# junwenxiong/diff_sal

Hardware: AMD Instinct MI355X
Metric: denoise-steps/sec (batch x NFE / wall time), 16x224x384 clip, 50-step DPM-Solver (higher is better)
Workload: dtype f32; 1 GPU; BASELINE configs[1]: DHF1k visual-only, batch=4/GPU, 224x384, 50-NFE DPM-Solver (multistep-2, logSNR, denoise-to-zero), faithful full graph; batch_per_gpu=4, nfe_per_trajectory=50, step=one SalUNet evaluation + DPM-Solver update on one batch, sampler_mode=eager

## Files before the change

diff_sal_amd/csrc/common.h:

```cpp
#pragma once
#include <hip/hip_runtime.h>

#include <cstdarg>
#include <cstdint>
#include <cstdio>

#include "../../include/diffsal.h"

namespace diffsal {

void set_error(const char* fmt, ...);
void note_kernel(const char* fmt, ...);

inline bool aligned16(const void* p) { return (reinterpret_cast<uintptr_t>(p) & 15u) == 0; }

inline int check_launch(const char* what) {
  hipError_t e = hipGetLastError();
  if (e != hipSuccess) {
    set_error("%s: launch failed: %s", what, hipGetErrorString(e));
    return DIFFSAL_E_LAUNCH;
  }
  return DIFFSAL_OK;
}

#define DS_REQUIRE(cond, code, ...)  \
  do {                               \
    if (!(cond)) {                   \
      diffsal::set_error(__VA_ARGS__); \
      return (code);                 \
    }                                \
  } while (0)

constexpr int kWave = 64;

#define DIFFSAL_TUNE_KEYS(X) \
  X(NO_PERSIST) X(NO_XCD_ORDER) X(NO_HALO) X(FORCE_HALO) X(IGEMM_CFG) X(IGEMM16_CFG) X(PLAN_DEBUG) \
  X(WGRAD_CFG) X(WGRAD_SPLITS) X(WGRAD_VERBOSE) X(NO_FUSED_BLOCK) X(NO_WINOGRAD) X(FORCE_WINOGRAD) X(GN_CHUNKS) \
  X(GN_APPLY_WGS) X(GEMM_DMA) X(CONV_DMA) X(GROUP_GRID) X(GEMM_DMA16) X(WGRAD_DMA) X(NO_GN_SLAB) X(NO_WINOGRAD4) X(BATCH_TILE) \
  X(BATCH_XCD) X(NO_TAPSUM_ROWS) X(TAPSUM_ROWS_FORM) X(NO_ATTN_BWD_DS) X(NO_POOL_RUNS) X(NO_ATTN_SLOTS) X(NO_STREAM16) \
  X(CONV16_TILE) X(BLOCK16_WAVES) X(NO_ATTN16_MFMA) X(CONV16_HALF) X(FRONT_FOLD_WGS)
#define DIFFSAL_TUNE_ENUM(name) TUNE_##name,
enum TuneKey { DIFFSAL_TUNE_KEYS(DIFFSAL_TUNE_ENUM) TUNE_COUNT };
#undef DIFFSAL_TUNE_ENUM
int tune(int key);

template <int CTRL>
__device__ __forceinline__ float dpp_move(float v) {
  return __builtin_bit_cast(float, __builtin_amdgcn_update_dpp(0, __builtin_bit_cast(int, v), CTRL, 0xF, 0xF, false));
}
__device__ __forceinline__ float lane_xor16(float v) {
  const unsigned u = __builtin_bit_cast(unsigned, v);
  const auto r = __builtin_amdgcn_permlane16_swap(u, u, false, false);
  return __builtin_bit_cast(float, (__lane_id() & 16) ? r[0] : r[1]);
}
__device__ __forceinline__ float lane_xor32(float v) {
  const unsigned u = __builtin_bit_cast(unsigned, v);
  const auto r = __builtin_amdgcn_permlane32_swap(u, u, false, false);
  return __builtin_bit_cast(float, (__lane_id() & 32) ? r[0] : r[1]);
}
template <int WIDTH, typename OP>
__device__ __forceinline__ float group_reduce(float v, OP op) {
  static_assert(WIDTH >= 1 && WIDTH <= 64 && (WIDTH & (WIDTH - 1)) == 0, "power of two <= 64");
  if constexpr (WIDTH >= 2) v = op(v, dpp_move<0xB1>(v));
  if constexpr (WIDTH >= 4) v = op(v, dpp_move<0x4E>(v));
  if constexpr (WIDTH >= 8) v = op(v, dpp_move<0x141>(v));
  if constexpr (WIDTH >= 16) v = op(v, dpp_move<0x140>(v));
  if constexpr (WIDTH >= 32) v = op(v, lane_xor16(v));
  if constexpr (WIDTH >= 64) v = op(v, lane_xor32(v));
  return v;
}
template <int WIDTH>
__device__ __forceinline__ float group_sum(float v) {
  return group_reduce<WIDTH>(v, [](float a, float b) { return a + b; });
// ... 295 lines not shown
```

diff_sal_amd/csrc/gemm_dma.hip:

```cpp
#include <type_traits>

#include "common.h"

namespace diffsal {

struct DmaGemmArgs {
  const void* a;
  const void* w;
  const float* bias;
  const float* scale;
  const float* shift;
  const float* rowvec;
  const void* residual;
  void* out;
  int M, N, K;
  int act, rowvec_ld, rows_per_img;
  int n_tiles_m, n_tiles_n, n_tiles;
  int xcd_order;
  int H, W, Cin, Ho, Wo, KW, taps, stride_h, stride_w, pad_t, pad_l, dil_h, dil_w;
  unsigned in_bytes;
  int splits, kt_per_unit;
  float* partial;
  int batch;
  long a_bs, w_bs, o_bs;
// ... 502 lines not shown
    stamp(3 + 3 * t);
    cmp_v += gsz;
  }
}

template <typename T>
__global__ __launch_bounds__(256) void gemm_dma_reduce_kernel(DmaGemmArgs p) {
  const T* __restrict__ resid = static_cast<const T*>(p.residual);
  T* __restrict__ outp = static_cast<T*>(p.out);
  const int n4 = p.N >> 2;
  const long total = static_cast<long>(p.M) * n4, slab = static_cast<long>(p.M) * p.N;
  for (long i = static_cast<long>(blockIdx.x) * 256 + threadIdx.x; i < total; i += static_cast<long>(gridDim.x) * 256) {
    const int n = static_cast<int>(i % n4) * 4;
    const long m = i / n4, o = m * p.N + n;
    float4 a = ld4(p.partial + o);
    for (int s = 1; s < p.splits; ++s) {
      const float4 b = ld4(p.partial + s * slab + o);
      a.x += b.x; a.y += b.y; a.z += b.z; a.w += b.w;
    }
    float v[4] = {a.x, a.y, a.z, a.w};
#pragma unroll
    for (int e = 0; e < 4; ++e) {
      float x[1] = {v[e]};
      epi_channels(x, p.bias, p.scale, p.shift, p.rowvec, [&] { return (m / p.rows_per_img) * p.rowvec_ld; }, n + e);
      epi_act(x, p.act);
      v[e] = x[0];
    }
    if (p.act == DIFFSAL_ACT_GELU_GRAD) epi_gelu_grad(v, ld4(resid + o));
    else if (resid) epi_add(v, ld4(resid + o));
    st4(outp + o, make_float4(v[0], v[1], v[2], v[3]));
  }
}

namespace {

int choose_split(long tiles, int kt, int stages, long mn, double* t_out = nullptr) {
  int best = 1;
  double best_t = 1e30;
  for (int S = 1; S <= 32; ++S) {
    if (kt % (S * stages) != 0) continue;
    const int per = kt / S;
    if (S > 1 && per < 2 * stages) break;
    const long units = tiles * S;
    const double rounds = static_cast<double>((units + 255) / 256);
    double t = rounds * per * 1.13e-6;
    t += 3.0e-6 + 1.2e-6;
    if (S > 1) t += (S + 1.0) * mn * 4.0 / 3.0e12 + 4.0e-6;
    if (t < best_t) { best_t = t; best = S; }
  }
  if (t_out) *t_out = best_t;
  return best;
}

template <typename T, int TMB, int TNB, int STAGES, int OCC>
int launch_dma(DmaGemmArgs& a, bool conv, hipStream_t s) {
  constexpr int BM = 32 * TMB, BN = 32 * TNB;
  const int slots = 256 * OCC;
  const int units = a.n_tiles * a.splits * (a.batch + a.batch2);
  const int grid = units < slots ? units : slots;
#ifdef DIFFSAL_DEV_STAMPS
  a.stamps = (g_dma_stamps && static_cast<size_t>(grid) * 32 * 8 <= g_dma_stamp_bytes) ? g_dma_stamps : nullptr;
#endif
  const long rows_total = static_cast<long>(a.n_tiles_m) * (a.batch + a.batch2);
  const bool batched = a.batch + a.batch2 > 1;
  a.xcd_order = (a.splits == 1 && tune(TUNE_NO_XCD_ORDER) != 1 && grid % 8 == 0 && a.n_tiles_n > 1 &&
                 (batched ? (tune(TUNE_BATCH_XCD) == 1 && units >= 128 && rows_total >= 16) : (a.n_tiles >= slots && a.n_tiles_m >= 16))) ? 1 : 0;
// ... 93 lines not shown
  else rc = launch_dma<f16_t, 3, 3, 3, 2>(g, false, s);
  return rc == DIFFSAL_OK ? 1 : rc;
}

int gemm_dma_batched(const float* a, const float* w, float* out, long M, int K, int N, int batch, long a_bs, long w_bs, long o_bs,
                     hipStream_t s, const float* side_a, const float* side_w, float* side_out, long side_rows) {
  diffsal_conv_desc d{};
  d.N = 1; d.H = 1; d.W = static_cast<int>(M); d.Ho = 1; d.Wo = static_cast<int>(M); d.Cin = K; d.Cout = N; d.KH = 1; d.KW = 1;
  d.stride_h = d.stride_w = d.dil_h = d.dil_w = 1;
  d.dtype = DIFFSAL_F32;
  if (M <= 0 || M >= (1L << 31) || batch < 1 || a_bs % 4 != 0 || w_bs % 4 != 0 || o_bs % 4 != 0) return 0;
  const long nb2 = side_rows > 0 ? side_rows / M : 0;
  if (side_rows > 0 && (side_rows % M != 0 || !side_a || !side_w || !side_out || !aligned16(side_a) || !aligned16(side_w) ||
                        !aligned16(side_out) || nb2 > 4096))
    return 0;
  const long tm = (M + 95) / 96, nbt = batch + nb2;
  const long u96 = tm * ((N + 95) / 96) * nbt, u128 = tm * ((N + 127) / 128) * nbt;
  const double t96 = static_cast<double>((u96 + 255) / 256), t128 = static_cast<double>((u128 + 255) / 256) * (4.0 / 3.0);
  const int force = tune(TUNE_BATCH_TILE);
  const bool wide = N % 128 == 0 && (force == 1 || (force != 0 && t128 * 1.1 < t96));
  DmaGemmArgs g;
  if (!dma_fill(g, kDmaCfgs[wide ? 2 : 0], &d, false, 4, a, w, nullptr, nullptr, nullptr, nullptr, 0, nullptr, out)) return 0;
  g.batch = batch; g.a_bs = a_bs; g.w_bs = w_bs; g.o_bs = o_bs;
  if (side_rows > 0) {
    g.batch2 = static_cast<int>(nb2);
    g.a2 = side_a; g.w2 = side_w; g.out2 = side_out;
    g.a2_bs = M * K; g.o2_bs = M * N;
  }
  if (static_cast<long>(g.n_tiles) * (batch + g.batch2) >= (1L << 30)) return 0;
  const int rc = wide ? launch_dma<float, 3, 4, 3, 1>(g, false, s) : launch_dma<float, 3, 3, 3, 2>(g, false, s);
  return rc == DIFFSAL_OK ? 1 : rc;
}

int try_gemm_dma_group(int n, const diffsal_conv_desc* const* d, const float* const* a, const float* const* w, const float* const* bias,
                       float* const* out, hipStream_t s) {
  if (n < 1 || n > kMaxGroup) return 0;
  const DmaCfg& c = kDmaCfgs[0];
  DmaGemmArgs pr[kMaxGroup];
  for (int i = 0; i < n; ++i)
    if (!dma_fill(pr[i], c, d[i], true, 4, a[i], w[i], bias ? bias[i] : nullptr, nullptr, nullptr, nullptr, 0, nullptr, out[i])) return 0;
  int order[kMaxGroup];
  for (int i = 0; i < n; ++i) order[i] = i;
  for (int i = 0; i < n; ++i)
    for (int j = i + 1; j < n; ++j)
      if (pr[order[j]].kt_per_unit > pr[order[i]].kt_per_unit) { const int t = order[i]; order[i] = order[j]; order[j] = t; }
  DmaGroupArgs g{};
  g.n = n;
  int units = 0;
  for (int i = 0; i < kMaxGroup; ++i) {
    if (i < n) {
      g.prob[i] = pr[order[i]];
      units += g.prob[i].n_tiles;
    } else {
      g.prob[i] = g.prob[n - 1];
    }
    g.unit_end[i] = i < n ? units : 0x7FFFFFFF;
  }
  g.total = units;
  const int persist = tune(TUNE_GROUP_GRID);
  const int grid = persist > 0 && units > persist ? persist : units;
  hipLaunchKernelGGL((gemm_dma_kernel<float, 3, 3, 3, 2, true, true>), dim3(grid), dim3(256), 0, s, g);
  note_kernel("gemm_dma_kernel<float, 3, 3, 3, 2, true, true> [96x96 tile, 3 stages, %d problems, %d units]", n, units);
  const int rc = check_launch("diffsal_conv_igemm_group(dma)");
  return rc == DIFFSAL_OK ? 1 : rc;
}

}

#ifdef DIFFSAL_DEV_STAMPS
extern "C" int diffsal_set_dma_stamps(void* device_buffer, size_t bytes) {
  diffsal::g_dma_stamps = static_cast<unsigned long long*>(device_buffer);
  diffsal::g_dma_stamp_bytes = device_buffer ? bytes : 0;
  return DIFFSAL_OK;
}
#endif
```

diff_sal_amd/csrc/igemm.hip:

```cpp
#include <cstdlib>
#include <type_traits>

#include "common.h"

namespace diffsal {

size_t igemm16_ws_bytes(const diffsal_conv_desc* d);
int igemm16_launch(const diffsal_conv_desc* d, const void* in, const void* w, const float* bias, const float* scale,
                   const float* shift, const float* rowvec, const void* residual, void* out, void* ws, size_t ws_bytes,
                   hipStream_t s, const void* in2 = nullptr, const void* w2 = nullptr, const float* bias2 = nullptr,
                   void* out2 = nullptr);

int try_linear_stream(const float* x, const float* w, const float* bias, const float* residual, float* out, long M,
                      int K, int N, int act, hipStream_t s);

int try_gemm_dma(int cfg, const diffsal_conv_desc* d, bool as_conv, const void* a, const void* w, const float* bias, const float* scale,
                 const float* shift, const float* rowvec, int rowvec_ld, const void* residual, void* out, void* ws, size_t ws_bytes,
                 hipStream_t s, bool out_f32 = false);
int try_gemm_dma_group(int n, const diffsal_conv_desc* const* d, const float* const* a, const float* const* w, const float* const* bias,
                       float* const* out, hipStream_t s);
size_t gemm_dma_ws_bytes(int cfg, long M, int K, int N, int esz);
int try_gemm16_dma2(const diffsal_conv_desc* d, const void* a, const void* w, const float* bias, const float* scale, const float* shift,
                    const float* rowvec, int rowvec_ld, const void* residual, void* out, hipStream_t s, bool out_f32);
double gemm_dma_estimate(int cfg, long M, int K, int N);

struct IgemmArgs {
  const float* in;
  const float* w;
  const float* bias;
  const float* scale;
  const float* shift;
  const float* rowvec;
  const float* residual;
  float* out;
  int M, K;
  int H, W, Cin, Ho, Wo, Cout;
  int KW, taps, stride_h, stride_w, pad_t, pad_l, dil_h, dil_w;
  int act, rowvec_ld;
  int linear;
  int persist_wgs;
  int w_split;
  int n_tiles_n, n_tiles;
  unsigned in_bytes, w_bytes;
  int splits, kt_per_split;
  float* partial;
  int vec_epilogue;
  int xcd_order;
  int pair;
  const float* in2;
  const float* w2;
  const float* bias2;
  float* out2;
  float* partial2;
// ... 705 lines not shown
  g = g > 2048 ? 2048 : g;
  hipLaunchKernelGGL(splitk_reduce_kernel, dim3(static_cast<int>(g), nz), dim3(256), 0, s, a);
  return check_launch("diffsal_conv_igemm(split-K reduce)");
}

}

using namespace diffsal;

static int dma_route(const diffsal_conv_desc* d, bool linear, long M, int K, bool pair) {
  if (d->precision != DIFFSAL_PREC_FP32 || d->w_format != 0 || pair) return -1;
  if (d->dtype != DIFFSAL_F32) {
    if (!linear || tune(TUNE_IGEMM16_CFG) >= 0 || K % 192 != 0 || d->Cout % 4 != 0) return -1;
    const int forced = tune(TUNE_GEMM_DMA16);
    if (forced == 0) return -1;
    if (forced > 0) return forced == 2 ? 3 : 0;
    return ((M + 95) / 96) * ((d->Cout + 95) / 96) >= 192 ? 0 : -1;
  }
  if (tune(TUNE_IGEMM_CFG) >= 0) return -1;
  const long tiles96 = ((M + 95) / 96) * ((d->Cout + 95) / 96);
  if (linear) {
    const int forced = tune(TUNE_GEMM_DMA);
    if (forced == 0) return -1;
    if (forced > 0) return forced - 1;
    if (K % 96 != 0 || d->Cout % 4 != 0) return -1;
    const double t_dma = gemm_dma_estimate(0, M, K, d->Cout);
    const double t_tiled = choose_plan(M, d->Cout, K, d->precision, true).t;
    return t_dma <= 1.25 * t_tiled ? 0 : -1;
  }
  const int forced = tune(TUNE_CONV_DMA);
  if (forced == 0) return -1;
  if (forced > 0) return forced - 1;
  if (K % 96 != 0 || d->Cout % 4 != 0) return -1;
  return ((tiles96 >= 1024 && K <= 1024) || (M <= 400 && K >= 3072)) ? 0 : -1;
}

static int validate(const diffsal_conv_desc* d) {
  DS_REQUIRE(d, DIFFSAL_E_ARG, "conv_igemm: null descriptor");
  DS_REQUIRE(d->Cin > 0 && d->Cin % 32 == 0, DIFFSAL_E_SHAPE, "conv_igemm: Cin=%d must be a multiple of 32", d->Cin);
  DS_REQUIRE(d->N > 0 && d->H > 0 && d->W > 0 && d->Cout > 0 && d->KH > 0 && d->KW > 0 && d->stride_h > 0 &&
                 d->stride_w > 0 && d->dil_h > 0 && d->dil_w > 0,
             DIFFSAL_E_SHAPE, "conv_igemm: non-positive dimension");
  DS_REQUIRE(d->Ho > 0 && d->Wo > 0, DIFFSAL_E_SHAPE, "conv_igemm: empty output %dx%d", d->Ho, d->Wo);
  const long M = static_cast<long>(d->N) * d->Ho * d->Wo;
  DS_REQUIRE(M < (1L << 31) && M * d->Cout < (1L << 40), DIFFSAL_E_SHAPE, "conv_igemm: problem too large");
  DS_REQUIRE(d->KH * d->KW <= 32, DIFFSAL_E_SHAPE, "conv_igemm: at most 32 taps (KH*KW=%d)", d->KH * d->KW);
  DS_REQUIRE(d->precision == DIFFSAL_PREC_FP32 || d->precision == DIFFSAL_PREC_BF16X3, DIFFSAL_E_ARG,
             "conv_igemm: precision %d (DIFFSAL_PREC_FP32 or DIFFSAL_PREC_BF16X3)", d->precision);
  DS_REQUIRE(d->dtype == DIFFSAL_F32 || d->dtype == DIFFSAL_BF16 || d->dtype == DIFFSAL_F16, DIFFSAL_E_ARG,
             "conv_igemm: dtype %d (DIFFSAL_F32, DIFFSAL_BF16 or DIFFSAL_F16)", d->dtype);
  DS_REQUIRE(d->dtype == DIFFSAL_F32 || (d->precision == DIFFSAL_PREC_FP32 && d->w_format == 0), DIFFSAL_E_ARG,
             "conv_igemm: 16-bit storage uses the native MFMA (precision and w_format must be 0)");
  const long esz = d->dtype == DIFFSAL_F32 ? 4 : 2;
  const long in_bytes = static_cast<long>(d->N) * d->H * d->W * d->Cin * esz;
  const long w_bytes = static_cast<long>(d->Cout) * d->KH * d->KW * d->Cin * esz;
  DS_REQUIRE(in_bytes < (1L << 32) - 16 && w_bytes < (1L << 32) - 16, DIFFSAL_E_SHAPE,
             "conv_igemm: input (%ld B) and weight (%ld B) must each stay below 4 GiB (32-bit buffer offsets); "
             "split the batch", in_bytes, w_bytes);
  return DIFFSAL_OK;
}

static Plan plan_or_forced(long M, int Cout, int K, int precision, bool linear) {
  Plan pl = choose_plan(M, Cout, K, precision, linear);
  const int v = tune(TUNE_IGEMM_CFG);
  if (v >= 0) {
    pl.cfg = (v % 8) % kNumCfgs;
    pl.splits = 1;
// ... 111 lines not shown
  a.kt_per_split = (a.K / BK + pl.splits - 1) / pl.splits;
  a.partial = nullptr;
  if (pl.splits > 1) {
    const size_t one = static_cast<size_t>(pl.splits) * M * d->Cout * sizeof(float);
    const size_t need = px ? 2 * one : one;
    DS_REQUIRE(ws && ws_bytes >= need && aligned16(ws) && aligned16(out), DIFFSAL_E_ARG,
               "conv_igemm: split-K needs %zu bytes of 16-byte aligned workspace (diffsal_conv_igemm_ws_bytes), got %zu",
               need, ws_bytes);
    a.partial = static_cast<float*>(ws);
    a.partial2 = px ? a.partial + one / sizeof(float) : nullptr;
  }
  a.vec_epilogue = d->Cout % 4 == 0 && aligned16(out) && (!residual || aligned16(residual)) && (!bias || aligned16(bias)) &&
                   (!scale || (aligned16(scale) && aligned16(shift))) && (!rowvec || (aligned16(rowvec) && a.rowvec_ld % 4 == 0));
  if (px) a.vec_epilogue = a.vec_epilogue && aligned16(px->out2) && (!px->bias2 || aligned16(px->bias2));
  a.persist_wgs = kCUs * kCfgs[pl.cfg].occ;
  if (tune(TUNE_NO_PERSIST) == 1) a.persist_wgs = 0;
  switch (pl.cfg) {
    case 0: return launch<2, 2, 2, 3>(a, s, d->precision);
    case 1: return launch<2, 2, 2, 2>(a, s, d->precision);
    case 2: return launch<4, 1, 1, 3>(a, s, d->precision);
    case 3: return launch<2, 2, 1, 2>(a, s, d->precision);
    case 4: return launch<2, 2, 2, 1>(a, s, d->precision);
    default: return launch<2, 2, 1, 1>(a, s, d->precision);
  }
}

extern "C" int diffsal_conv_igemm(const diffsal_conv_desc* d, const void* in_v, const void* w_v,
                                  const float* bias, const float* scale, const float* shift,
                                  const float* rowvec, const void* residual_v, void* out_v, void* ws,
                                  size_t ws_bytes, diffsal_stream_t stream) {
  return conv_igemm_impl(d, in_v, w_v, bias, scale, shift, rowvec, residual_v, out_v, ws, ws_bytes, stream, nullptr);
}

extern "C" int diffsal_conv_igemm_group(int n, const diffsal_conv_desc* const* descs, const void* const* in, const void* const* w,
                                        const float* const* bias, void* const* out, void* ws, size_t ws_bytes, diffsal_stream_t stream) {
  DS_REQUIRE(n >= 1 && n <= 4 && descs && in && w && out, DIFFSAL_E_ARG, "conv_igemm_group: 1..4 problems, non-null tables");
  bool dma_ok = tune(TUNE_GEMM_DMA) != 0 && tune(TUNE_IGEMM_CFG) < 0;
  for (int i = 0; i < n; ++i) {
    const int rc = validate(descs[i]);
    if (rc) return rc;
    DS_REQUIRE(in[i] && w[i] && out[i], DIFFSAL_E_ARG, "conv_igemm_group: null operand of problem %d", i);
    DS_REQUIRE(descs[i]->act >= DIFFSAL_ACT_NONE && descs[i]->act <= DIFFSAL_ACT_SIGMOID, DIFFSAL_E_ARG, "conv_igemm_group: act=%d", descs[i]->act);
    dma_ok = dma_ok && descs[i]->dtype == DIFFSAL_F32 && descs[i]->precision == DIFFSAL_PREC_FP32 && descs[i]->w_format == 0;
  }
  if (dma_ok) {
    const float* a_[4]; const float* w_[4]; const float* b_[4]; float* o_[4];
    for (int i = 0; i < n; ++i) {
      a_[i] = static_cast<const float*>(in[i]); w_[i] = static_cast<const float*>(w[i]);
      b_[i] = bias ? bias[i] : nullptr; o_[i] = static_cast<float*>(out[i]);
    }
    const int r = try_gemm_dma_group(n, descs, a_, w_, b_, o_, static_cast<hipStream_t>(stream));
    if (r != 0) return r < 0 ? r : DIFFSAL_OK;
  }
  for (int i = 0; i < n; ++i) {
    const int rc = conv_igemm_impl(descs[i], in[i], w[i], bias ? bias[i] : nullptr, nullptr, nullptr, nullptr, nullptr, out[i], ws, ws_bytes,
                                   stream, nullptr);
    if (rc) return rc;
  }
  return DIFFSAL_OK;
}

extern "C" int diffsal_linear_f32out(const diffsal_conv_desc* d, const void* in, const void* w, const float* bias, float* out,
                                     diffsal_stream_t stream) {
  DS_REQUIRE(d && in && w && out, DIFFSAL_E_ARG, "linear_f32out: null argument");
  int rc = validate(d);
  if (rc) return rc;
  DS_REQUIRE(is_linear(d) && d->dtype != DIFFSAL_F32 && d->precision == DIFFSAL_PREC_FP32 && d->w_format == 0 &&
                 d->act >= DIFFSAL_ACT_NONE && d->act <= DIFFSAL_ACT_SIGMOID,
             DIFFSAL_E_ARG, "linear_f32out: a plain product on bf16 / f16 storage");
  DS_REQUIRE(aligned16(in) && aligned16(w) && aligned16(out) && (!bias || aligned16(bias)), DIFFSAL_E_ALIGN, "linear_f32out: misaligned pointer");
  int rr = try_gemm16_dma2(d, in, w, bias, nullptr, nullptr, nullptr, d->Cout, nullptr, out, static_cast<hipStream_t>(stream), true);
  if (rr == 0)
    rr = try_gemm_dma(0, d, false, in, w, bias, nullptr, nullptr, nullptr, d->Cout, nullptr, out, nullptr, 0,
                      static_cast<hipStream_t>(stream), true);
  if (rr < 0) return rr;
  DS_REQUIRE(rr == 1, DIFFSAL_E_SHAPE, "linear_f32out: K=%d must be a multiple of 192 and N=%d of 4", d->KH * d->KW * d->Cin, d->Cout);
  return DIFFSAL_OK;
}

extern "C" int diffsal_linear_pair(const diffsal_conv_desc* d, const void* in0, const void* in1, const void* w0, const void* w1,
                                   const float* bias0, const float* bias1, void* out0, void* out1, void* ws, size_t ws_bytes,
                                   diffsal_stream_t stream) {
  DS_REQUIRE(d && in0 && in1 && w0 && w1 && out0 && out1, DIFFSAL_E_ARG, "linear_pair: null argument");
  DS_REQUIRE(d->KH == 1 && d->KW == 1 && d->stride_h == 1 && d->stride_w == 1 && d->pad_t == 0 && d->pad_l == 0 &&
                 d->Ho == d->H && d->Wo == d->W && d->act == DIFFSAL_ACT_NONE && d->w_format == 0 && d->precision == DIFFSAL_PREC_FP32,
             DIFFSAL_E_SHAPE, "linear_pair: two plain [M,K] x [K,N] products of one shape (1x1, no activation, exact arithmetic)");
  DS_REQUIRE((bias0 == nullptr) == (bias1 == nullptr), DIFFSAL_E_ARG, "linear_pair: both products carry a bias or neither does");
  DS_REQUIRE(aligned16(in1) && aligned16(w1), DIFFSAL_E_ALIGN, "linear_pair: in/w must be 16-byte aligned");
  {
    const long M = static_cast<long>(d->N) * d->Ho * d->Wo;
    const long tiles = 2 * ((M + 95) / 96) * ((d->Cout + 95) / 96);
    if (d->dtype == DIFFSAL_F32 && tiles >= 192 && tune(TUNE_GEMM_DMA) != 0 && tune(TUNE_IGEMM_CFG) < 0) {
      const int rv = validate(d);
      if (rv) return rv;
      const diffsal_conv_desc* dd[2] = {d, d};
      const float* a_[2] = {static_cast<const float*>(in0), static_cast<const float*>(in1)};
      const float* w_[2] = {static_cast<const float*>(w0), static_cast<const float*>(w1)};
      const float* b_[2] = {bias0, bias1};
      float* o_[2] = {static_cast<float*>(out0), static_cast<float*>(out1)};
      const int r = try_gemm_dma_group(2, dd, a_, w_, b_, o_, static_cast<hipStream_t>(stream));
      if (r != 0) return r < 0 ? r : DIFFSAL_OK;
    }
  }
  const PairExtra px{in1, w1, bias1, out1};
  return conv_igemm_impl(d, in0, w0, bias0, nullptr, nullptr, nullptr, nullptr, out0, ws, ws_bytes, stream, &px);
}
```

diff_sal_amd/ops.py:

```python
from __future__ import annotations

import contextlib
import ctypes as C
import threading
from typing import List, Optional, Sequence, Tuple

import torch

from . import _lib
from ._lib import ACT_GELU, ACT_GELU_GRAD, ACT_NONE, ACT_RELU, ACT_SIGMOID, ConvDesc

Tensor = torch.Tensor

PROFILE = None


_PROF_DEPTH = [0]


class _prof:
    __slots__ = ("cls", "flops", "nbytes", "e0", "note", "counted", "kernel")

    def __init__(self, cls, flops=0.0, nbytes=0.0, note="", kernel=""):
        self.cls, self.flops, self.nbytes, self.e0, self.note, self.counted = cls, float(flops), float(nbytes), None, note, False
# ... 600 lines not shown
        return out
    ws_bytes = lib.diffsal_conv_igemm_ws_bytes(C.byref(d))
    ws = torch.empty((ws_bytes // 4,), device=x.device, dtype=torch.float32) if ws_bytes else None
    with _prof(tag, 2.0 * N * Ho * Wo * Cout * kh * kw * Cin, _nb(x, w_packed, residual, out),
               f"M={N * Ho * Wo} K={kh * kw * Cin} N={Cout} {kh}x{kw}" if PROFILE is not None else "") as pr:
        _lib.check(lib.diffsal_conv_igemm(C.byref(d), _pa(x, dt), _pa(w_packed, dt), _p(bias), _p(scale), _p(shift), rv,
                                          _pa(residual, dt), _pa(out, dt), _p(ws), ws_bytes, _stream()), "conv_igemm")
        if PROFILE is not None:
            pr.kernel = lib.diffsal_last_gemm_kernel().decode()
    return out


def up2_conv3x3_d2(z: Tensor, w_packed: Tensor, wino, tapw: Tensor, *, scale: Optional[Tensor] = None, shift: Optional[Tensor] = None,
                   act: int = ACT_NONE, tag: str = "K12", ring_only: bool = False):
    lib = _lib.load()
    N, h, w, Cin = z.shape
    Cout = w_packed.shape[0]
    c_ext = conv_igemm(z, w_packed, kh=3, kw=3, pad=(2, 2), dil=(1, 1), out_hw=(h + 2, w + 2), tag=tag, wino=wino)
    z = z.contiguous()
    zb = torch.empty((N, 2 * w + 2 * h - 4, Cin), device=z.device, dtype=z.dtype)
    dt = _dt(z)
    _lib.check(lib.diffsal_border_gather(_pa(z, dt), _pa(zb, dt), N, h, w, Cin, dt, _stream()), "border_gather")
    tb = linear(zb, tapw, None, tag=tag)
    out = torch.empty((N, 2 * h, 2 * w, Cout), device=z.device, dtype=z.dtype)
    with _prof(tag + "-tap", 0.0, _nb(c_ext, tb) + (0 if ring_only else _nb(out)),
               f"up2 commute {h}x{w} C={Cout}" + (" (border ring only)" if ring_only else "") if PROFILE is not None else "") as pr:
        dt = _dt(z)
        fn = lib.diffsal_up2_conv_commute_ring if ring_only else lib.diffsal_up2_conv_commute
        _lib.check(fn(_pa(c_ext, dt), _pa(tb, dt), _p(scale), _p(shift), _pa(out, dt), N, h, w, Cout, act, dt, _stream()), "up2_conv_commute")
        pr.kernel = "up2_conv_commute_ring_kernel" if ring_only else "up2_conv_commute_kernel"
    return (out, c_ext) if ring_only else out


def conv_igemm_group(problems: Sequence[dict], tag: str = "gemm") -> List[Tensor]:
    lib = _lib.load()
    n = len(problems)
    if not 1 <= n <= 4:
        raise RuntimeError("conv_igemm_group: 1..4 problems")
    if get_gemm_precision() != "fp32" or any(getattr(pr["w"], "_diffsal_split", False) for pr in problems):
        return [conv_igemm(pr["x"], pr["w"], kh=pr.get("kh", 1), kw=pr.get("kw", 1), stride=pr.get("stride", (1, 1)),
                           pad=pr.get("pad", (0, 0)), dil=pr.get("dil", (1, 1)), out_hw=pr.get("out_hw"), bias=pr.get("bias"),
                           act=pr.get("act", ACT_NONE), out=pr.get("out"), tag=tag) for pr in problems]
    descs, outs, keep = [], [], []
    flops = nbytes = 0.0
    ws_bytes = 0
    notes = []
    for pr in problems:
        x, w = pr["x"], pr["w"]
        kh, kw = pr.get("kh", 1), pr.get("kw", 1)
        stride, pad, dil = pr.get("stride", (1, 1)), pr.get("pad", (0, 0)), pr.get("dil", (1, 1))
        N, H, W, Cin = x.shape
        Cout = w.shape[0]
        assert w.shape[1] == kh * kw * Cin, (w.shape, kh, kw, Cin)
        if pr.get("out_hw") is None:
            Ho = (H + 2 * pad[0] - dil[0] * (kh - 1) - 1) // stride[0] + 1
            Wo = (W + 2 * pad[1] - dil[1] * (kw - 1) - 1) // stride[1] + 1
        else:
            Ho, Wo = pr["out_hw"]
        dt = _dt(x)
        out = pr.get("out")
        if out is None:
            out = torch.empty((N, Ho, Wo, Cout), device=x.device, dtype=x.dtype)
        d = ConvDesc(N, H, W, Cin, Ho, Wo, Cout, kh, kw, stride[0], stride[1], pad[0], pad[1], dil[0], dil[1], pr.get("act", ACT_NONE),
                     0, 0, _lib.PREC_FP32, dt)
        descs.append(d)
        outs.append(out)
        ws_bytes = max(ws_bytes, lib.diffsal_conv_igemm_ws_bytes(C.byref(d)))
        flops += 2.0 * N * Ho * Wo * Cout * kh * kw * Cin
        nbytes += _nb(x, w, out)
        notes.append(f"M={N * Ho * Wo} K={kh * kw * Cin} N={Cout} {kh}x{kw}")
    ws = torch.empty((ws_bytes // 4,), device=outs[0].device, dtype=torch.float32) if ws_bytes else None
    PA = C.c_void_p * n
    dp = (C.POINTER(ConvDesc) * n)(*[C.pointer(d) for d in descs])
    xs = PA(*[_pa(pr["x"], _dt(pr["x"])) for pr in problems])
    wsl = PA(*[_pa(pr["w"], _dt(pr["x"])) for pr in problems])
    bs = PA(*[_p(pr.get("bias")) for pr in problems])
    os_ = PA(*[_pa(o, _dt(o)) for o in outs])
    keep.extend([dp, xs, wsl, bs, os_])
    with _prof(tag, flops, nbytes, "group: " + " | ".join(notes) if PROFILE is not None else "") as pr_:
        _lib.check(lib.diffsal_conv_igemm_group(n, C.cast(dp, C.c_void_p), C.cast(xs, C.c_void_p), C.cast(wsl, C.c_void_p),
                                                C.cast(bs, C.c_void_p), C.cast(os_, C.c_void_p), _p(ws), ws_bytes, _stream()),
                   "conv_igemm_group")
        if PROFILE is not None:
            pr_.kernel = lib.diffsal_last_gemm_kernel().decode()
    return outs


def linear(x: Tensor, w: Tensor, bias: Optional[Tensor] = None, *, act: int = ACT_NONE,
           residual: Optional[Tensor] = None, tag: str = "K10", out_f32: bool = False) -> Tensor:
    lead = x.shape[:-1]
    M = 1
    for s in lead:
        M *= s
    if out_f32:
        if x.dtype == torch.float32 or residual is not None:
            raise RuntimeError("linear(out_f32=True): 16-bit storage in, no residual")
        lib = _lib.load()
        K, N = x.shape[-1], w.shape[0]
        dt = _dt(x)
        d = ConvDesc(1, 1, M, K, 1, M, N, 1, 1, 1, 1, 0, 0, 1, 1, act, 0, 0, _lib.PREC_FP32, dt)
        out = torch.empty((M, N), device=x.device, dtype=torch.float32)
        xc = x.reshape(M, K)
        with _prof(tag, 2.0 * M * N * K, _nb(xc, w, out), f"M={M} K={K} N={N} 1x1 (fp32 out)" if PROFILE is not None else "") as pr:
            _lib.check(lib.diffsal_linear_f32out(C.byref(d), _pa(xc, dt), _pa(w, dt), _p(bias), _p(out), _stream()), "linear_f32out")
            if PROFILE is not None:
                pr.kernel = lib.diffsal_last_gemm_kernel().decode()
# ... 1596 lines not shown
```

diff_sal_amd/sal_unet.py:

```python
from __future__ import annotations

import contextlib
import math
from typing import Dict, List, Optional, Sequence

import torch
from torch import nn

from . import ops
from .ops import ACT_GELU, ACT_NONE, ACT_RELU

Tensor = torch.Tensor


def _holder(**children) -> nn.Module:
    m = nn.Module()
    for k, v in children.items():
        setattr(m, k, v)
    return m


def _seq_named(pairs) -> nn.Sequential:
    from collections import OrderedDict

# ... 678 lines not shown
                    u, _, _ = ops.conv3x3_wino4_ex(u, pk[f"s{i}.pe2.wino"].f4, scale=pk[f"s{i}.pe2.scale"], shift=pk[f"s{i}.pe2.shift"],
                                                   act=ACT_RELU, residual=None if skip is None else skip.view(Bn * T, 2 * h, 2 * w, C),
                                                   dil=2, up2=fuse_up, tag="K12")
                else:
                    u = ops.conv_igemm(u, pk[f"s{i}.pe2.w"], kh=3, kw=3, pad=(d, d), dil=(d, d),
                                       scale=pk[f"s{i}.pe2.scale"], shift=pk[f"s{i}.pe2.shift"], act=ACT_RELU, tag="K12",
                                       residual=None if skip is None else skip.view(Bn * T, 2 * h, 2 * w, C),
                                       wino=pk[f"s{i}.pe2.wino"])
                xcur = u.view(Bn, T, 2 * h, 2 * w, C)
            kt = self.temporal_list[i]
            if (xcur.shape[1] - kt) // kt + 1 != 1:
                raise RuntimeError(f"ReduceTemp: T={xcur.shape[1]}, kernel/stride {kt} must give exactly one frame")
            nm = dec.norm_mts[i]
            xcur, z = self._block(i, xcur, pk, audio_tok, audio_hw, norm_z=nm)
            if taps is not None:
                taps[f"stage{i}"] = xcur
            Bn, T, H, W, _ = xcur.shape
            if z is None:
                z = ops.layernorm(xcur, nm.weight, nm.bias, nm.eps)
            z_out = None
            if z_all is not None:
                if (H, W) != sizes[i]:
                    raise RuntimeError(f"stage {i}: {H}x{W} tokens, expected {sizes[i]}")
                z_out = z_all[z_off:z_off + Bn * H * W].view(Bn, 1, H * W, self.ori_embed_dim)
                z_off += Bn * H * W
            if z_out is not None and self.group_reduce_temp and cdt == torch.float32:
                redu.append(dict(x=z.view(Bn, T, H * W, C), w=pk[f"s{i}.redu.w"], kh=kt, kw=1, stride=(kt, 1), act=ACT_RELU, out=z_out))
                zs.append(z_out.view(Bn, H, W, self.ori_embed_dim))
                continue
            z = ops.conv_igemm(z.view(Bn, T, H * W, C), pk[f"s{i}.redu.w"], kh=kt, kw=1, stride=(kt, 1), act=ACT_RELU,
                               out=z_out, tag="K13")
            zs.append(z.view(Bn, H, W, self.ori_embed_dim))
        if redu:
            def _units(pr):
                n, t, hw, c = pr["x"].shape
                return -(-n * hw // 96) * -(-pr["w"].shape[0] // 96), pr["kh"] * c // 32
            while len(redu) > 1:
                work = sum(u * k for u, k in map(_units, redu)) / 256.0
                j = max(range(len(redu)), key=lambda q: _units(redu[q])[1])
                if _units(redu[j])[1] <= 1.5 * work:
                    break
                pr = redu.pop(j)
                ops.conv_igemm(pr["x"], pr["w"], kh=pr["kh"], kw=pr["kw"], stride=pr["stride"], act=pr["act"], out=pr["out"], tag="K13")
            ops.conv_igemm_group(redu, tag="K13")
        mt = dec.mt_proj
        if z_all is not None:
            f32_taps = cdt != torch.float32 and self.mt_tap16_f32 and "mt" not in self.tap_conv16 and self.ori_embed_dim % 192 == 0
            y9 = ops.linear(z_all, pk["mt.tapw"], None, tag="K14", out_f32=f32_taps)
            ys, off = [], 0
            for z_ in zs:
                m_ = z_.shape[0] * z_.shape[1] * z_.shape[2]
                ys.append(y9[off:off + m_].view(z_.shape[0], z_.shape[1], z_.shape[2], y9.shape[-1]))
                off += m_
            if self.fold_head and mt[0].out_channels <= 128 and mt[0].out_channels % 4 == 0:
                s = ops.tapsum(ys, th, tw, mt[0].out_channels, dil=1, bias=mt[0].bias, scale=pk["mt.scale"], shift=pk["mt.shift"],
                               act=ACT_RELU, tag="K14-tap", head=(pk["head.w"], self.logits.linear_pred.bias))
                if lowres:
                    return s
                out = ops.resize_bilinear(s, self.img_size[0], self.img_size[1], tag="K14-head")
                return out.view(B, 1, self.img_size[0], self.img_size[1])
            y = ops.tapsum(ys, th, tw, mt[0].out_channels, dil=1, bias=mt[0].bias, scale=pk["mt.scale"], shift=pk["mt.shift"],
                           act=ACT_RELU, tag="K14-tap")
        else:
            acc = ops.resize_sum(zs, th, tw)
            if taps is not None:
                taps["multi_scale"] = acc
            y = ops.conv_igemm(acc, pk["mt.w"], kh=3, kw=3, pad=(1, 1), bias=mt[0].bias, scale=pk["mt.scale"],
                               shift=pk["mt.shift"], act=ACT_RELU, tag="K14")
        s = ops.head_sigmoid(y, pk["head.w"], self.logits.linear_pred.bias)
        if lowres:
            return s
        out = ops.resize_bilinear(s, self.img_size[0], self.img_size[1], tag="K14-head")
        return out.view(B, 1, self.img_size[0], self.img_size[1])

    dropout_p = 0.1
    _dropout_calls = 0
# ... 177 lines not shown
```

include/diffsal.h:

```cpp
#ifndef DIFFSAL_H
#define DIFFSAL_H

#include <stddef.h>
#include <stdint.h>

#ifdef __cplusplus
extern "C" {
#endif

typedef void* diffsal_stream_t;

enum {
  DIFFSAL_OK = 0,
  DIFFSAL_E_SHAPE = -1,
  DIFFSAL_E_ALIGN = -2,
  DIFFSAL_E_LAUNCH = -3,
  DIFFSAL_E_ARG = -4
};

enum { DIFFSAL_ACT_NONE = 0, DIFFSAL_ACT_RELU = 1, DIFFSAL_ACT_GELU_ERF = 2, DIFFSAL_ACT_SIGMOID = 3,
       DIFFSAL_ACT_GELU_GRAD = 5 };

#define DIFFSAL_ABI_VERSION 51
int diffsal_version(void);
// ... 84 lines not shown
int diffsal_conv_wino4_stages(const diffsal_conv_desc* d , const float* x, const float* U, const float* bias,
                              const float* scale, const float* shift, const float* rowvec, const float* residual, float* out,
                              void* ws, size_t ws_bytes, int stages, diffsal_stream_t stream);
typedef struct diffsal_wino4_ext {
  const float* in_ab;
  const float* side_a;
  const float* side_w;
  float* side_out;
  double* out_stats;
  const float* up2_c;
  const float* up2_scale;
  const float* up2_shift;
  long long side_rows;
  int in_swish;
  int out_groups;
  int up2_act;
  int reserved;
} diffsal_wino4_ext;
size_t diffsal_conv_wino4_stats_bytes(const diffsal_conv_desc* d , int groups);
int diffsal_conv_wino4_side_supported(const diffsal_conv_desc* d , long side_rows);
int diffsal_conv_wino4_ex(const diffsal_conv_desc* d , const float* x, const float* U, const float* bias,
                          const float* scale, const float* shift, const float* rowvec, const float* residual, float* out,
                          void* ws, size_t ws_bytes, const diffsal_wino4_ext* ext , int stages,
                          diffsal_stream_t stream);
int diffsal_gn_affine(const void* x, const float* gamma, const float* beta, float* ab, int B, int HW, int C, int groups,
                      float eps, void* ws, size_t ws_bytes, int dtype, diffsal_stream_t stream);
int diffsal_gn_affine_wino4(const diffsal_conv_desc* d , const double* stats, const float* gamma, const float* beta,
                            int groups, float eps, float* ab, diffsal_stream_t stream);
int diffsal_border_gather(const void* z, void* zb, int N, int h, int w, int C, int dtype, diffsal_stream_t stream);
int diffsal_up2_conv_commute(const void* c_ext, const void* tap_border, const float* scale, const float* shift, void* out,
                             int N, int h, int w, int C, int act, int dtype, diffsal_stream_t stream);
int diffsal_up2_conv_commute_ring(const void* c_ext, const void* tap_border, const float* scale, const float* shift, void* out,
                             int N, int h, int w, int C, int act, int dtype, diffsal_stream_t stream);
int diffsal_conv_igemm_group(int n, const diffsal_conv_desc* const* descs, const void* const* in, const void* const* w,
                             const float* const* bias, void* const* out, void* ws, size_t ws_bytes, diffsal_stream_t stream);

int diffsal_linear_pair(const diffsal_conv_desc* d, const void* in0, const void* in1, const void* w0, const void* w1,
                        const float* bias0, const float* bias1, void* out0, void* out1, void* ws, size_t ws_bytes,
                        diffsal_stream_t stream);


int diffsal_col2im_disjoint(const float* cols, float* dx, int N, int H, int W, int C, int Ho, int Wo, int KH, int KW,
                            int stride_h, int stride_w, int pad_t, int pad_l, diffsal_stream_t stream);
int diffsal_col2im_gather(const float* cols, float* dx, int N, int H, int W, int C, int Ho, int Wo, int KH, int KW,
                          int stride_h, int stride_w, int pad_t, int pad_l, diffsal_stream_t stream);
int diffsal_pack_weight(const float* src, float* dst, int Cout, int Cin, int taps, int mode, diffsal_stream_t stream);
typedef struct diffsal_pack_job {
  const void* src;
  void* dst;
  int Cout, Cin, taps, mode;
  int tile0, reserved;
} diffsal_pack_job;
int diffsal_pack_weight_many(const diffsal_pack_job* jobs_dev , int n_jobs, int total_tiles, int max_taps,
                             diffsal_stream_t stream);
int diffsal_split_weight(const float* src, float* dst, long n, diffsal_stream_t stream);

size_t diffsal_conv_wgrad_ws_bytes(const diffsal_conv_desc* d );
int diffsal_conv_wgrad_splits(const diffsal_conv_desc* d );
int diffsal_conv_wgrad(const diffsal_conv_desc* d , const float* in, const float* dy, float* dw_packed,
                       double* dbias_part, float* dbias_out, void* ws, size_t ws_bytes, diffsal_stream_t stream);
size_t diffsal_wgrad_segmented_ws_bytes(int segments, int seg_rows, int K, int Cout);
int diffsal_wgrad_segmented(const float* x, const float* dy, float* out, int segments, int seg_rows, int K, int Cout,
                            void* ws, size_t ws_bytes, diffsal_stream_t stream);
int diffsal_colsum(const float* dy, float* out, int M, int C, int seg_rows, void* ws, size_t ws_bytes,
                   diffsal_stream_t stream);

// ... 287 lines not shown
```

Baseline: 1262 denoise-steps/s.

## Add per-problem split-K to grouped DMA GEMM with fused reduction kernel

Grouped implicit-GEMM launches can now split K per problem, using a planner that balances the longest unit's K loop against total work. Partial slabs go to a workspace sized by a new ws-size API, and a separate grouped sum kernel reduces them and applies bias and activation. This replaces the Python heuristic that pulled long-K problems out of the group into separate launches, aiming to cut tail imbalance and launch count. It adds an extra reduction pass and workspace traffic, and tightens the single-GEMM DMA selection condition.

```diff
diff --git a/diff_sal_amd/csrc/common.h b/diff_sal_amd/csrc/common.h
--- a/diff_sal_amd/csrc/common.h
+++ b/diff_sal_amd/csrc/common.h
@@ -38,7 +38,7 @@
   X(WGRAD_CFG) X(WGRAD_SPLITS) X(WGRAD_VERBOSE) X(NO_FUSED_BLOCK) X(NO_WINOGRAD) X(FORCE_WINOGRAD) X(GN_CHUNKS) \
   X(GN_APPLY_WGS) X(GEMM_DMA) X(CONV_DMA) X(GROUP_GRID) X(GEMM_DMA16) X(WGRAD_DMA) X(NO_GN_SLAB) X(NO_WINOGRAD4) X(BATCH_TILE) \
   X(BATCH_XCD) X(NO_TAPSUM_ROWS) X(TAPSUM_ROWS_FORM) X(NO_ATTN_BWD_DS) X(NO_POOL_RUNS) X(NO_ATTN_SLOTS) X(NO_STREAM16) \
-  X(CONV16_TILE) X(BLOCK16_WAVES) X(NO_ATTN16_MFMA) X(CONV16_HALF) X(FRONT_FOLD_WGS)
+  X(CONV16_TILE) X(BLOCK16_WAVES) X(NO_ATTN16_MFMA) X(CONV16_HALF) X(FRONT_FOLD_WGS) X(GROUP_SPLIT)
 #define DIFFSAL_TUNE_ENUM(name) TUNE_##name,
 enum TuneKey { DIFFSAL_TUNE_KEYS(DIFFSAL_TUNE_ENUM) TUNE_COUNT };
 #undef DIFFSAL_TUNE_ENUM
diff --git a/diff_sal_amd/csrc/gemm_dma.hip b/diff_sal_amd/csrc/gemm_dma.hip
--- a/diff_sal_amd/csrc/gemm_dma.hip
+++ b/diff_sal_amd/csrc/gemm_dma.hip
@@ -558,6 +558,42 @@
   }
 }
 
+struct DmaGroupSumArgs {
+  long end4[kMaxGroup];
+  const float* partial[kMaxGroup];
+  const float* bias[kMaxGroup];
+  float* out[kMaxGroup];
+  long slab[kMaxGroup];
+  int N[kMaxGroup], splits[kMaxGroup], act[kMaxGroup];
+};
+
+__global__ __launch_bounds__(256) void gemm_dma_group_sum_kernel(DmaGroupSumArgs g) {
+  const long total = g.end4[kMaxGroup - 1];
+  for (long i = static_cast<long>(blockIdx.x) * 256 + threadIdx.x; i < total; i += static_cast<long>(gridDim.x) * 256) {
+    const int idx = (i >= g.end4[0]) + (i >= g.end4[1]) + (i >= g.end4[2]);
+#define DS_PICK(f) (idx == 0 ? g.f[0] : idx == 1 ? g.f[1] : idx == 2 ? g.f[2] : g.f[3])
+    const long li = i - (idx == 0 ? 0 : idx == 1 ? g.end4[0] : idx == 2 ? g.end4[1] : g.end4[2]);
+    const float* __restrict__ partial = DS_PICK(partial);
+    const float* __restrict__ bias = DS_PICK(bias);
+    float* __restrict__ outp = DS_PICK(out);
+    const long slab = DS_PICK(slab);
+    const int N = DS_PICK(N), splits = DS_PICK(splits), act = DS_PICK(act);
+#undef DS_PICK
+    const int n4 = N >> 2;
+    const int n = static_cast<int>(li % n4) * 4;
+    const long o = (li / n4) * N + n;
+    float4 a = ld4(partial + o);
+    for (int s = 1; s < splits; ++s) {
+      const float4 b = ld4(partial + s * slab + o);
+      a.x += b.x; a.y += b.y; a.z += b.z; a.w += b.w;
+    }
+    float v[4] = {a.x, a.y, a.z, a.w};
+    epi_channels(v, bias, nullptr, nullptr, nullptr, n);
+    epi_act(v, act);
+    st4(outp + o, make_float4(v[0], v[1], v[2], v[3]));
+  }
+}
+
 namespace {
 
 int choose_split(long tiles, int kt, int stages, long mn, double* t_out = nullptr) {
@@ -717,36 +753,143 @@
   return rc == DIFFSAL_OK ? 1 : rc;
 }
 
+namespace {
+
+struct GroupPlan { int splits[kMaxGroup]; size_t ws_bytes; };
+
+bool group_split_ok(int kt, int S, int stages) { return S == 1 || (kt % (S * stages) == 0 && kt / S >= 2 * stages); }
+
+GroupPlan plan_group(int n, const DmaGemmArgs* pr, int stages) {
+  GroupPlan best{};
+  for (int i = 0; i < kMaxGroup; ++i) best.splits[i] = 1;
+  const int forced = tune(TUNE_GROUP_SPLIT);
+  if (forced == 0) return best;
+  if (forced > 1) {
+    for (int i = 0; i < n; ++i)
+      if (group_split_ok(pr[i].kt_per_unit, forced, stages)) best.splits[i] = forced;
+  } else {
+    double total = 0.0;
+    for (int i = 0; i < n; ++i) total += static_cast<double>(pr[i].n_tiles) * pr[i].kt_per_unit;
+    double best_t = 1e30;
+    int S[kMaxGroup] = {1, 1, 1, 1};
+    auto cost = [&]() {
+      long units = 0;
+      int longest = 0;
+      double slabs = 0.0;
+      bool any = false;
+      for (int i = 0; i < n; ++i) {
+        units += static_cast<long>(pr[i].n_tiles) * S[i];
+        const int per = pr[i].kt_per_unit / S[i];
+        longest = per > longest ? per : longest;
+        if (S[i] > 1) { any = true; slabs += (S[i] + 1.0) * pr[i].M * pr[i].N * 4.0 / 3.0e12; }
+      }
+      const double t_unit = longest * (units > 256 ? 2.2e-6 : 1.13e-6);
+      const double t_work = total * 1.34e-6 / 256.0;
+      return (t_unit > t_work ? t_unit : t_work) + slabs + (any ? 4.0e-6 : 0.0);
+    };
+    for (int L = 1 << 30; L > 0;) {
+      int next = 0;
+      for (int i = 0; i < n; ++i) {
+        S[i] = 1;
+        for (int sp = 1; sp <= 32; ++sp) {
+          if (!group_split_ok(pr[i].kt_per_unit, sp, stages)) continue;
+          const int per = pr[i].kt_per_unit / sp;
+          if (per < L && per > next) next = per;
+          if (pr[i].kt_per_unit / S[i] > L) S[i] = sp;
+        }
+      }
+      const double t = cost();
+      if (t < best_t * (1.0 - 1e-9)) { best_t = t; for (int j = 0; j < n; ++j) best.splits[j] = S[j]; }
+      L = next;
+    }
+  }
+  for (int i = 0; i < n; ++i)
+    if (best.splits[i] > 1) best.ws_bytes += static_cast<size_t>(best.splits[i]) * pr[i].M * pr[i].N * sizeof(float);
+  return best;
+}
+
+bool group_fill(int n, const diffsal_conv_desc* const* d, const float* const* a, const float* const* w, const float* const* bias,
+                float* const* out, DmaGemmArgs* pr) {
+  if (n < 1 || n > kMaxGroup) return false;
+  for (int i = 0; i < n; ++i)
+    if (!dma_fill(pr[i], kDmaCfgs[0], d[i], true, 4, a[i], w[i], bias ? bias[i] : nullptr, nullptr, nullptr, nullptr, 0, nullptr, out[i]))
+      return false;
+  return true;
+}
+
+}
+
+size_t gemm_dma_group_ws_bytes(int n, const diffsal_conv_desc* const* d) {
+  DmaGemmArgs pr[kMaxGroup];
+  const float* al[kMaxGroup];
+  float* ol[kMaxGroup];
+  for (int i = 0; i < kMaxGroup; ++i) { al[i] = reinterpret_cast<const float*>(16); ol[i] = reinterpret_cast<float*>(16); }
+  if (!group_fill(n, d, al, al, nullptr, ol, pr)) return 0;
+  return plan_group(n, pr, kDmaCfgs[0].stages).ws_bytes;
+}
+
 int try_gemm_dma_group(int n, const diffsal_conv_desc* const* d, const float* const* a, const float* const* w, const float* const* bias,
-                       float* const* out, hipStream_t s) {
-  if (n < 1 || n > kMaxGroup) return 0;
+                       float* const* out, void* ws, size_t ws_bytes, hipStream_t s) {
   const DmaCfg& c = kDmaCfgs[0];
   DmaGemmArgs pr[kMaxGroup];
-  for (int i = 0; i < n; ++i)
-    if (!dma_fill(pr[i], c, d[i], true, 4, a[i], w[i], bias ? bias[i] : nullptr, nullptr, nullptr, nullptr, 0, nullptr, out[i])) return 0;
+  if (!group_fill(n, d, a, w, bias, out, pr)) return 0;
+  const GroupPlan plan = plan_group(n, pr, c.stages);
+  if (plan.ws_bytes > 0 && ws && aligned16(ws) && ws_bytes >= plan.ws_bytes) {
+    float* slab = static_cast<float*>(ws);
+    for (int i = 0; i < n; ++i) {
+      if (plan.splits[i] == 1) continue;
+      pr[i].splits = plan.splits[i];
+      pr[i].kt_per_unit /= plan.splits[i];
+      pr[i].partial = slab;
+      slab += static_cast<size_t>(plan.splits[i]) * pr[i].M * pr[i].N;
+    }
+  }
   int order[kMaxGroup];
   for (int i = 0; i < n; ++i) order[i] = i;
   for (int i = 0; i < n; ++i)
     for (int j = i + 1; j < n; ++j)
       if (pr[order[j]].kt_per_unit > pr[order[i]].kt_per_unit) { const int t = order[i]; order[i] = order[j]; order[j] = t; }
   DmaGroupArgs g{};
+  DmaGroupSumArgs sum{};
   g.n = n;
-  int units = 0;
+  long units = 0, sum4 = 0;
+  int n_split = 0;
   for (int i = 0; i < kMaxGroup; ++i) {
     if (i < n) {
       g.prob[i] = pr[order[i]];
-      units += g.prob[i].n_tiles;
+      units += static_cast<long>(g.prob[i].n_tiles) * g.prob[i].splits;
+      if (g.prob[i].splits > 1) {
+        const DmaGemmArgs& p = g.prob[i];
+        const long mn = static_cast<long>(p.M) * p.N;
+        sum4 += mn / 4;
+        sum.partial[n_split] = p.partial; sum.bias[n_split] = p.bias; sum.out[n_split] = static_cast<float*>(p.out);
+        sum.slab[n_split] = mn; sum.N[n_split] = p.N; sum.splits[n_split] = p.splits; sum.act[n_split] = p.act;
+        sum.end4[n_split] = sum4;
+        ++n_split;
+      }
     } else {
       g.prob[i] = g.prob[n - 1];
     }
-    g.unit_end[i] = i < n ? units : 0x7FFFFFFF;
-  }
-  g.total = units;
+    g.unit_end[i] = i < n ? static_cast<int>(units) : 0x7FFFFFFF;
+  }
+  if (units >= (1L << 30)) return 0;
+  for (int i = n_split; i < kMaxGroup; ++i) {
+    sum.end4[i] = sum4;
+    sum.partial[i] = nullptr; sum.bias[i] = nullptr; sum.out[i] = nullptr; sum.slab[i] = 0; sum.N[i] = 4; sum.splits[i] = 1; sum.act[i] = 0;
+  }
+  g.total = static_cast<int>(units);
   const int persist = tune(TUNE_GROUP_GRID);
-  const int grid = persist > 0 && units > persist ? persist : units;
+  const int grid = persist > 0 && units > persist ? persist : static_cast<int>(units);
   hipLaunchKernelGGL((gemm_dma_kernel<float, 3, 3, 3, 2, true, true>), dim3(grid), dim3(256), 0, s, g);
-  note_kernel("gemm_dma_kernel<float, 3, 3, 3, 2, true, true> [96x96 tile, 3 stages, %d problems, %d units]", n, units);
-  const int rc = check_launch("diffsal_conv_igemm_group(dma)");
+  note_kernel("gemm_dma_kernel<float, 3, 3, 3, 2, true, true> [96x96 tile, 3 stages, %d problems, %d units, split-K %d/%d/%d/%d]", n,
+              static_cast<int>(units), g.prob[0].splits, n > 1 ? g.prob[1].splits : 0, n > 2 ? g.prob[2].splits : 0, n > 3 ? g.prob[3].splits : 0);
+  int rc = check_launch("diffsal_conv_igemm_group(dma)");
+  if (rc == DIFFSAL_OK && n_split > 0) {
+    long gs = (sum4 + 255) / 256;
+    gs = gs > 2048 ? 2048 : gs;
+    hipLaunchKernelGGL(gemm_dma_group_sum_kernel, dim3(static_cast<unsigned>(gs)), dim3(256), 0, s, sum);
+    rc = check_launch("diffsal_conv_igemm_group(dma split-K sum)");
+  }
   return rc == DIFFSAL_OK ? 1 : rc;
 }
 
diff --git a/diff_sal_amd/csrc/igemm.hip b/diff_sal_amd/csrc/igemm.hip
--- a/diff_sal_amd/csrc/igemm.hip
+++ b/diff_sal_amd/csrc/igemm.hip
@@ -18,7 +18,8 @@
                  const float* shift, const float* rowvec, int rowvec_ld, const void* residual, void* out, void* ws, size_t ws_bytes,
                  hipStream_t s, bool out_f32 = false);
 int try_gemm_dma_group(int n, const diffsal_conv_desc* const* d, const float* const* a, const float* const* w, const float* const* bias,
-                       float* const* out, hipStream_t s);
+                       float* const* out, void* ws, size_t ws_bytes, hipStream_t s);
+size_t gemm_dma_group_ws_bytes(int n, const diffsal_conv_desc* const* d);
 size_t gemm_dma_ws_bytes(int cfg, long M, int K, int N, int esz);
 int try_gemm16_dma2(const diffsal_conv_desc* d, const void* a, const void* w, const float* bias, const float* scale, const float* shift,
                     const float* rowvec, int rowvec_ld, const void* residual, void* out, hipStream_t s, bool out_f32);
@@ -790,7 +791,7 @@
   if (forced == 0) return -1;
   if (forced > 0) return forced - 1;
   if (K % 96 != 0 || d->Cout % 4 != 0) return -1;
-  return ((tiles96 >= 1024 && K <= 1024) || (M <= 400 && K >= 3072)) ? 0 : -1;
+  return ((tiles96 >= 1024 && K <= 1024) || (M <= 400 && K >= 3072 && tiles96 >= 32)) ? 0 : -1;
 }
 
 static int validate(const diffsal_conv_desc* d) {
@@ -968,24 +969,44 @@
   return conv_igemm_impl(d, in_v, w_v, bias, scale, shift, rowvec, residual_v, out_v, ws, ws_bytes, stream, nullptr);
 }
 
+static bool group_takes_dma(int n, const diffsal_conv_desc* const* descs) {
+  bool ok = tune(TUNE_GEMM_DMA) != 0 && tune(TUNE_IGEMM_CFG) < 0;
+  for (int i = 0; i < n; ++i)
+    ok = ok && descs[i]->dtype == DIFFSAL_F32 && descs[i]->precision == DIFFSAL_PREC_FP32 && descs[i]->w_format == 0;
+  return ok;
+}
+
+extern "C" size_t diffsal_conv_igemm_group_ws_bytes(int n, const diffsal_conv_desc* const* descs) {
+  if (n < 1 || n > 4 || !descs) return 0;
+  size_t need = 0;
+  for (int i = 0; i < n; ++i) {
+    if (validate(descs[i]) != DIFFSAL_OK) return 0;
+    const size_t one = diffsal_conv_igemm_ws_bytes(descs[i]);
+    need = one > need ? one : need;
+  }
+  if (group_takes_dma(n, descs)) {
+    const size_t g = gemm_dma_group_ws_bytes(n, descs);
+    need = g > need ? g : need;
+  }
+  return need;
+}
+
 extern "C" int diffsal_conv_igemm_group(int n, const diffsal_conv_desc* const* descs, const void* const* in, const void* const* w,
                                         const float* const* bias, void* const* out, void* ws, size_t ws_bytes, diffsal_stream_t stream) {
   DS_REQUIRE(n >= 1 && n <= 4 && descs && in && w && out, DIFFSAL_E_ARG, "conv_igemm_group: 1..4 problems, non-null tables");
-  bool dma_ok = tune(TUNE_GEMM_DMA) != 0 && tune(TUNE_IGEMM_CFG) < 0;
   for (int i = 0; i < n; ++i) {
     const int rc = validate(descs[i]);
     if (rc) return rc;
     DS_REQUIRE(in[i] && w[i] && out[i], DIFFSAL_E_ARG, "conv_igemm_group: null operand of problem %d", i);
     DS_REQUIRE(descs[i]->act >= DIFFSAL_ACT_NONE && descs[i]->act <= DIFFSAL_ACT_SIGMOID, DIFFSAL_E_ARG, "conv_igemm_group: act=%d", descs[i]->act);
-    dma_ok = dma_ok && descs[i]->dtype == DIFFSAL_F32 && descs[i]->precision == DIFFSAL_PREC_FP32 && descs[i]->w_format == 0;
-  }
-  if (dma_ok) {
+  }
+  if (group_takes_dma(n, descs)) {
     const float* a_[4]; const float* w_[4]; const float* b_[4]; float* o_[4];
     for (int i = 0; i < n; ++i) {
       a_[i] = static_cast<const float*>(in[i]); w_[i] = static_cast<const float*>(w[i]);
       b_[i] = bias ? bias[i] : nullptr; o_[i] = static_cast<float*>(out[i]);
     }
-    const int r = try_gemm_dma_group(n, descs, a_, w_, b_, o_, static_cast<hipStream_t>(stream));
+    const int r = try_gemm_dma_group(n, descs, a_, w_, b_, o_, ws, ws_bytes, static_cast<hipStream_t>(stream));
     if (r != 0) return r < 0 ? r : DIFFSAL_OK;
   }
   for (int i = 0; i < n; ++i) {
@@ -1034,7 +1055,7 @@
       const float* w_[2] = {static_cast<const float*>(w0), static_cast<const float*>(w1)};
       const float* b_[2] = {bias0, bias1};
       float* o_[2] = {static_cast<float*>(out0), static_cast<float*>(out1)};
-      const int r = try_gemm_dma_group(2, dd, a_, w_, b_, o_, static_cast<hipStream_t>(stream));
+      const int r = try_gemm_dma_group(2, dd, a_, w_, b_, o_, nullptr, 0, static_cast<hipStream_t>(stream));
       if (r != 0) return r < 0 ? r : DIFFSAL_OK;
     }
   }
diff --git a/diff_sal_amd/ops.py b/diff_sal_amd/ops.py
--- a/diff_sal_amd/ops.py
+++ b/diff_sal_amd/ops.py
@@ -656,7 +656,7 @@
     return (out, c_ext) if ring_only else out
 
 
-def conv_igemm_group(problems: Sequence[dict], tag: str = "gemm") -> List[Tensor]:
+def conv_igemm_group(problems: Sequence[dict], tag: str = "gemm", ws: Optional[Tensor] = None) -> List[Tensor]:
     lib = _lib.load()
     n = len(problems)
     if not 1 <= n <= 4:
@@ -667,7 +667,6 @@
                            act=pr.get("act", ACT_NONE), out=pr.get("out"), tag=tag) for pr in problems]
     descs, outs, keep = [], [], []
     flops = nbytes = 0.0
-    ws_bytes = 0
     notes = []
     for pr in problems:
         x, w = pr["x"], pr["w"]
@@ -689,13 +688,17 @@
                      0, 0, _lib.PREC_FP32, dt)
         descs.append(d)
         outs.append(out)
-        ws_bytes = max(ws_bytes, lib.diffsal_conv_igemm_ws_bytes(C.byref(d)))
         flops += 2.0 * N * Ho * Wo * Cout * kh * kw * Cin
         nbytes += _nb(x, w, out)
         notes.append(f"M={N * Ho * Wo} K={kh * kw * Cin} N={Cout} {kh}x{kw}")
-    ws = torch.empty((ws_bytes // 4,), device=outs[0].device, dtype=torch.float32) if ws_bytes else None
     PA = C.c_void_p * n
     dp = (C.POINTER(ConvDesc) * n)(*[C.pointer(d) for d in descs])
+    if ws is not None:
+        assert ws.dtype == torch.float32 and ws.is_contiguous() and ws.is_cuda
+        ws_bytes = ws.numel() * 4
+    else:
+        ws_bytes = lib.diffsal_conv_igemm_group_ws_bytes(n, C.cast(dp, C.c_void_p))
+        ws = torch.empty((ws_bytes // 4,), device=outs[0].device, dtype=torch.float32) if ws_bytes else None
     xs = PA(*[_pa(pr["x"], _dt(pr["x"])) for pr in problems])
     wsl = PA(*[_pa(pr["w"], _dt(pr["x"])) for pr in problems])
     bs = PA(*[_p(pr.get("bias")) for pr in problems])
diff --git a/diff_sal_amd/sal_unet.py b/diff_sal_amd/sal_unet.py
--- a/diff_sal_amd/sal_unet.py
+++ b/diff_sal_amd/sal_unet.py
@@ -734,16 +734,6 @@
                                out=z_out, tag="K13")
             zs.append(z.view(Bn, H, W, self.ori_embed_dim))
         if redu:
-            def _units(pr):
-                n, t, hw, c = pr["x"].shape
-                return -(-n * hw // 96) * -(-pr["w"].shape[0] // 96), pr["kh"] * c // 32
-            while len(redu) > 1:
-                work = sum(u * k for u, k in map(_units, redu)) / 256.0
-                j = max(range(len(redu)), key=lambda q: _units(redu[q])[1])
-                if _units(redu[j])[1] <= 1.5 * work:
-                    break
-                pr = redu.pop(j)
-                ops.conv_igemm(pr["x"], pr["w"], kh=pr["kh"], kw=pr["kw"], stride=pr["stride"], act=pr["act"], out=pr["out"], tag="K13")
             ops.conv_igemm_group(redu, tag="K13")
         mt = dec.mt_proj
         if z_all is not None:
diff --git a/include/diffsal.h b/include/diffsal.h
--- a/include/diffsal.h
+++ b/include/diffsal.h
@@ -140,6 +140,7 @@
                              int N, int h, int w, int C, int act, int dtype, diffsal_stream_t stream);
 int diffsal_up2_conv_commute_ring(const void* c_ext, const void* tap_border, const float* scale, const float* shift, void* out,
                              int N, int h, int w, int C, int act, int dtype, diffsal_stream_t stream);
+size_t diffsal_conv_igemm_group_ws_bytes(int n, const diffsal_conv_desc* const* descs );
 int diffsal_conv_igemm_group(int n, const diffsal_conv_desc* const* descs, const void* const* in, const void* const* w,
                              const float* const* bias, void* const* out, void* ws, size_t ws_bytes, diffsal_stream_t stream);
 
```

Result: no change. 1262 denoise-steps/s, median of 2 (-0.0%).
